# bjing2016/mdgen

Measured on AMD Instinct MI355X. Metric: sampled MD frames/sec, higher is better.
Workload: dtype bf16; 1 GPU; tetrapeptide_fwdsim_crop4_T1000_B16; batch_per_gpu=16, num_frames=1000, crop=4, euler_steps=49, hipgraph=True, parallelism=batch-sharded x1, no collective

## Files before the change

### mdgen_amd/csrc/k_gemm.hip

```cpp
#include "kernels.h"
#include "panel.h"

namespace mdg {

constexpr int kRowB = kC * 2;
constexpr int kPanelBytes = kPanel * kRowB;

constexpr int kRopeLds = kRopeRow + 4;
constexpr int kBiasUnits = 3 * kC / 4;
struct QkvStage {
    float bias[3][kC];
    float rope[kPanel][kRopeLds];
};
struct Attn4Stage {
    float bias[3][kC];
    uint32_t tab[2][kL4Tab];
    float rope[4][kRopeLds];
};
__device__ __forceinline__ const f32x4* stage_bias_src(const QkvParams& p, int u) {
    const float* b = u < kC / 4 ? p.bq : u < 2 * (kC / 4) ? p.bk : p.bv;
    return reinterpret_cast<const f32x4*>(b) + (u % (kC / 4));
}
template <int NT>
struct QkvStager {
// ... 296 lines not shown
        prologue_bf16<kC>(panel, pr, p.obuf);
        __syncthreads();
        wave_gemm<2, 3, 24, false, 4, true>(panel, kRowB, 0, 0, p.wo + (size_t)(3 * w) * 24 * 64 + lane, 24 * 64, acc);
        __syncthreads();
        epilogue_gate_residual_lds<3>(acc, pr, reinterpret_cast<float*>(panel) + w * (32 * 96), 96 * w, p.bo, p.mm, p.gate_chunk,
                                      true, p.h_rw);
        __syncthreads();
    }
    prologue_ln<false>(panel, pr, PRE ? p.h_rw : p.h, p.mm, p.shift_chunk, p.scale_chunk, 1e-6f);
    __syncthreads();
    QKV_STAMP(1);
    const int ntile = p.ax.ntile();
    const int len = p.ax.len;
    wave_gemm<2, 3, 24, true, 4, true>(panel, kRowB, 0, 0, p.wq + (size_t)(3 * w) * 24 * 64 + lane, 24 * 64, acc);
    QKV_STAMP(2);
    epilogue_heads_T<true, 2, !SMALL>(acc, pr, w, sbq, srope, SMALL, pos0, len, seq, ntile, tile0, p.qf, p.qkv_small, 0);
    __builtin_amdgcn_sched_barrier(0);
    QKV_STAMP(3);
    wave_gemm<2, 3, 24, true, 4, true>(panel, kRowB, 0, 0, p.wk + (size_t)(3 * w) * 24 * 64 + lane, 24 * 64, acc);
    QKV_STAMP(4);
    epilogue_heads_T<true, 2, !SMALL>(acc, pr, w, sbk, srope, SMALL, pos0, len, seq, ntile, tile0, p.kf, p.qkv_small, 1);
    __builtin_amdgcn_sched_barrier(0);
    QKV_STAMP(5);
    if (SMALL) {
        wave_gemm<2, 3, 24, true, 4, true>(panel, kRowB, 0, 0, p.wv + (size_t)(3 * w) * 24 * 64 + lane, 24 * 64, acc);
        epilogue_heads_T<false>(acc, pr, w, p.bv, nullptr, true, pos0, len, seq, ntile, tile0, nullptr, p.qkv_small, 2);
    } else {
        wave_gemm<2, 3, 24, false, 4, true>(panel, kRowB, 0, 0, p.wv + (size_t)(3 * w) * 24 * 64 + lane, 24 * 64, acc);
        QKV_STAMP(6);
        epilogue_v_flash(acc, w, sbv, seq, ntile, tile0, p.vf);
        if ((int)blockIdx.x - seq * p.panels_per_seq == p.panels_per_seq - 1) {
            __builtin_amdgcn_sched_barrier(0);
            write_bias_slots(p, seq, w);
        }
        QKV_STAMP(7);
    }
}

template <int J>
__device__ __forceinline__ float quad_bcast(float v) {
    return __builtin_bit_cast(float, __builtin_amdgcn_update_dpp(0, __builtin_bit_cast(int, v), J * 0x55, 0xf, 0xf, true));
}
template <int J>
__device__ __forceinline__ float fmac_dpp(float acc, float k, float q) {
    asm("v_fmac_f32_dpp %0, %1, %2 quad_perm:[%3,%3,%3,%3] row_mask:0xf bank_mask:0xf bound_ctrl:1" : "+v"(acc) : "v"(k), "v"(q), "n"(J));
    return acc;
}
template <int J>
__device__ __forceinline__ float mul_dpp(float k, float q) {
    float r;
    asm("v_mul_f32_dpp %0, %1, %2 quad_perm:[%3,%3,%3,%3] row_mask:0xf bank_mask:0xf bound_ctrl:1" : "=v"(r) : "v"(k), "v"(q), "n"(J));
    return r;
}
__device__ __forceinline__ void dpp_fence(float (&k)[12]) {
    asm volatile("s_nop 1"
                 : "+v"(k[0]), "+v"(k[1]), "+v"(k[2]), "+v"(k[3]), "+v"(k[4]), "+v"(k[5]), "+v"(k[6]), "+v"(k[7]), "+v"(k[8]), "+v"(k[9]),
                   "+v"(k[10]), "+v"(k[11]));
}
__device__ __forceinline__ float half_sum(float x) {
    const auto r = __builtin_amdgcn_permlane32_swap(__float_as_uint(x), __float_as_uint(x), false, false);
    return __uint_as_float(r[0]) + __uint_as_float(r[1]);
}
template <int TT = 2>
__device__ __forceinline__ void head_values(const f32x16* acc, int tt, int hd, const f32x4 (&bq)[3], float (&e)[12]) {
#pragma unroll
    for (int c = 0; c < 3; ++c) {
        const int ap = 3 * hd + c, ft = ap >> 2, a = ap & 3;
#pragma unroll
        for (int b = 0; b < 4; ++b) e[4 * c + b] = acc[ft * TT + tt][4 * a + b] + bq[c][b];
    }
}
template <bool X1S>
__device__ __forceinline__ void rotate_pair(float x1, float x2, float c, float sn, float& e0, float& e1) {
    const float a = x2 * sn;
    e0 = __builtin_fmaf(x1, c, -a);
    if (X1S) {
        const float b = x1 * sn;
        e1 = __builtin_fmaf(x2, c, b);
    } else {
        const float b = x2 * c;
        e1 = __builtin_fmaf(x1, sn, b);
    }
}
__device__ __forceinline__ void load_head_bias(const float* bias_perm, int w, int hh, f32x4 (&bq)[4][3]) {
    const f32x4* bp = reinterpret_cast<const f32x4*>(bias_perm + (w * 2 + hh) * 48);
#pragma unroll
    for (int hd = 0; hd < 4; ++hd)
#pragma unroll
        for (int c = 0; c < 3; ++c) bq[hd][c] = bp[hd * 3 + c];
}


template <bool SPLIT, bool HALF = false>
__global__ __launch_bounds__(512, 1) void k_ln_qkv8(const QkvParams p) {
    static_assert(!HALF || SPLIT, "32-row workgroups exist in the split form only");
    constexpr int TT = HALF ? 1 : 2, kRows = 32 * TT;
    __shared__ __attribute__((aligned(16))) unsigned char smem[sizeof(PanelRows) + kPanelBytes];
    __shared__ __attribute__((aligned(16))) QkvStage stage;
    QkvStager<512> stager;
    PanelRows* pr = reinterpret_cast<PanelRows*>(smem);
    unsigned char* panel = smem + sizeof(PanelRows);
    const int blk = SPLIT ? blockIdx.x >> 1 : blockIdx.x, half = SPLIT ? blockIdx.x & 1 : 0;
    const int seq = blk / p.panels_per_seq;
    const int pn = blk - seq * p.panels_per_seq;
    const int pos0 = pn * kRows, tile0 = pn * TT;
    stager.load(p, pos0, p.ax.len, threadIdx.x);
    setup_rows_axis(pr, p.ax, seq, pos0, p.mm, kRows);
    if (wave_id() == 0 && half == 0) {
        const int lane = lane_id(), len = p.ax.len, pos = pos0 + lane;
        const float mv = p.mk.at(p.ax.token(seq, pos < len ? pos : len - 1));
        const unsigned long long bal = __ballot(pos == len || (pos < len && mv != 0.f));
        uint32_t* vm = p.vmask + (long)seq * p.vmask_stride;
        if (lane < TT) vm[tile0 + lane] = (uint32_t)(bal >> (32 * lane));
        if (pn == p.panels_per_seq - 1) {
            const int idx = tile0 + TT + lane;
            if (idx < p.vmask_stride) vm[idx] = idx == (len >> 5) ? 1u << (len & 31) : 0u;
            if (idx + 64 < p.vmask_stride) vm[idx + 64] = 0u;
        }
    }
    __syncthreads();
    stager.store(&stage, threadIdx.x);
    const int w8 = __builtin_amdgcn_readfirstlane(wave_id()), g = w8 >> 2, w = w8 & 3, lane = lane_id();
    if (HALF) {
        if (g == 0) prologue_ln<false, 0, 1>(panel, pr, p.h, p.mm, p.shift_chunk, p.scale_chunk, 1e-6f, w, lane);
        else prologue_ln<false, 1, 2>(panel, pr, p.h, p.mm, p.shift_chunk, p.scale_chunk, 1e-6f, w, lane);
    } else {
        if (g == 0) prologue_ln<false, 0, 2>(panel, pr, p.h, p.mm, p.shift_chunk, p.scale_chunk, 1e-6f, w, lane);
        else prologue_ln<false, 2, 4>(panel, pr, p.h, p.mm, p.shift_chunk, p.scale_chunk, 1e-6f, w, lane);
    }
    __syncthreads();
    const int ntile = p.ax.ntile(), len = p.ax.len;
    const bool last = pn == p.panels_per_seq - 1;
    f32x16 acc[3 * TT];
    const bool do_q = SPLIT ? half == 0 && g == 0 : g == 0, do_k = SPLIT ? half == 0 && g == 1 : g == 0;
    const bool do_v = SPLIT ? half == 1 && g == 0 : g == 1;
    if (do_q) {
        wave_gemm<TT, 3, 24, true, 4, true>(panel, kRowB, 0, 0, p.wq + (size_t)(3 * w) * 24 * 64 + lane, 24 * 64, acc);
        epilogue_heads_T<true, TT, true>(acc, pr, w, stage.bias[0], &stage.rope[0][0], false, pos0, len, seq, ntile, tile0, p.qf, p.qkv_small, 0);
        __builtin_amdgcn_sched_barrier(0);
    }
    if (do_k) {
        wave_gemm<TT, 3, 24, true, 4, true>(panel, kRowB, 0, 0, p.wk + (size_t)(3 * w) * 24 * 64 + lane, 24 * 64, acc);
        epilogue_heads_T<true, TT, true>(acc, pr, w, stage.bias[1], &stage.rope[0][0], false, pos0, len, seq, ntile, tile0, p.kf, p.qkv_small, 1);
        if (last) {
            __builtin_amdgcn_sched_barrier(0);
            write_bias_slots(p, seq, w, true, false, TT);
        }
    }
    if (do_v) {
        wave_gemm<TT, 3, 24, false, 4, true>(panel, kRowB, 0, 0, p.wv + (size_t)(3 * w) * 24 * 64 + lane, 24 * 64, acc);
        epilogue_v_flash<TT>(acc, w, stage.bias[2], seq, ntile, tile0, p.vf);
        if (last) {
            __builtin_amdgcn_sched_barrier(0);
            write_bias_slots(p, seq, w, false, true, TT);
        }
    }
}

constexpr int kAttn4KPF = 2, kAttn4VPF = 3;
template <bool PROJ, bool HALF = false>
__global__ __launch_bounds__(256, 2) void k_ln_qkv_attn4(const QkvParams p) {
    static_assert(!HALF || PROJ, "the half-panel form is the whole sub-layer");
    constexpr int TT = HALF ? 1 : 2, kRows = HALF ? 32 : kPanel;
    __shared__ __attribute__((aligned(16))) unsigned char smem[sizeof(PanelRows) + kPanelBytes];
    __shared__ uint32_t qstash[HALF ? 1 : 4][24][64];
    __shared__ __attribute__((aligned(16))) Attn4Stage stage;
    Attn4Stager stager;
    PanelRows* pr = reinterpret_cast<PanelRows*>(smem);
    unsigned char* panel = smem + sizeof(PanelRows);
    ATTN4_STAMP_DECL;
    ATTN4_STAMP(0);
    stager.load(p, threadIdx.x);
    {
        const long row0 = (long)blockIdx.x * kRows, rend = row0 + kRows;
        setup_rows_linear(pr, row0, rend < p.nrows ? rend : p.nrows, p.mm);
    }
    __syncthreads();
    stager.store(&stage, threadIdx.x);
    const int w = __builtin_amdgcn_readfirstlane(wave_id());
    constexpr int t0 = 0;
    if (HALF) prologue_ln<false, 0, 2>(panel, pr, p.h, p.mm, p.shift_chunk, p.scale_chunk, 1e-6f, w, lane_id());
    else prologue_ln<false>(panel, pr, p.h, p.mm, p.shift_chunk, p.scale_chunk, 1e-6f);
    __syncthreads();
    ATTN4_STAMP(1);
    const int lane = lane_id(), hh = lane >> 5, tk = lane & 31;
    constexpr int L = 4;
    int tok[TT];
    float mval[TT];
#pragma unroll
    for (int tt = 0; tt < TT; ++tt) {
        tok[tt] = pr->tok[(t0 + tt) * 32 + tk];
        mval[tt] = p.mk.at(tok[tt] < 0 ? 0 : tok[tt]);
    }
    auto load_rope = [&](f32x4 (&rq)[TT][4]) {
#pragma unroll
        for (int tt = 0; tt < TT; ++tt) {
            const int tc = tok[tt] < 0 ? 0 : tok[tt];
            const f32x4* rc = reinterpret_cast<const f32x4*>(&stage.rope[tc & (L - 1)][16 * hh]);
#pragma unroll
            for (int i = 0; i < 4; ++i) rq[tt][i] = rc[i];
        }
    };
    f32x16 acc[3 * TT];
    f32x4 bb[4][3];
    f32x4 rq[TT][4];
    wave_gemm<TT, 3, 24, true, 4, true>(panel, kRowB, t0, 0, p.wq + (size_t)(3 * w) * 24 * 64 + lane, 24 * 64, acc);
    ATTN4_STAMP(2);
    load_head_bias(stage.bias[0], w, hh, bb);
    load_rope(rq);
    uint32_t qp[TT][4][6];
#pragma unroll
    for (int tt = 0; tt < TT; ++tt)
#pragma unroll
        for (int hd = 0; hd < 4; ++hd) {
            float e[12];
            head_values<TT>(acc, tt, hd, bb[hd], e);
#pragma unroll
            for (int q = 0; q < 6; ++q) {
                const float c = rq[tt][q >> 2][q & 3], sn = rq[tt][2 + (q >> 2)][q & 3];
                float r0, r1;
                rotate_pair<HALF>(e[2 * q], e[2 * q + 1], c, sn, r0, r1);
                qp[tt][hd][q] = pack_bf16(r0, r1);
            }
        }
    if constexpr (!HALF) {
#pragma unroll
        for (int hd = 0; hd < 4; ++hd)
#pragma unroll
            for (int q = 0; q < 6; ++q) qstash[w][hd * 6 + q][lane] = qp[TT - 1][hd][q];
    }
    ATTN4_STAMP(3);
    __builtin_amdgcn_sched_barrier(0);
    wave_gemm<TT, 3, 24, true, HALF ? 4 : kAttn4KPF, true>(panel, kRowB, t0, 0, p.wk + (size_t)(3 * w) * 24 * 64 + lane, 24 * 64, acc);
    ATTN4_STAMP(4);
    load_head_bias(stage.bias[1], w, hh, bb);
    load_rope(rq);
#pragma unroll
    for (int tt = 0; tt < TT; ++tt)
#pragma unroll
        for (int hd = 0; hd < 4; ++hd) {
            float k[12];
            head_values<TT>(acc, tt, hd, bb[hd], k);
#pragma unroll
            for (int c = 0; c < 3; ++c) {
                const int ap = 3 * hd + c, ft = ap >> 2, a = ap & 3;
#pragma unroll
                for (int b2 = 0; b2 < 2; ++b2) {
                    const int q = 2 * c + b2;
                    const float cs = rq[tt][q >> 2][q & 3], sn = rq[tt][2 + (q >> 2)][q & 3];
                    float r0, r1;
                    rotate_pair<HALF>(k[2 * q], k[2 * q + 1], cs, sn, r0, r1);
                    acc[ft * TT + tt][4 * a + 2 * b2] = r0;
                    acc[ft * TT + tt][4 * a + 2 * b2 + 1] = r1;
                }
            }
        }
    ATTN4_STAMP(5);
    __builtin_amdgcn_sched_barrier(0);
    float P[TT][4][5];
    {
#pragma unroll
        for (int hd = 0; hd < 4; ++hd) {
            const uint32_t* kt = &stage.tab[0][((2 * w + hh) * 4 + hd) * 6];
            float kb[12];
#pragma unroll
            for (int q = 0; q < 6; ++q) {
                kb[2 * q] = bf16_lo(kt[q]);
                kb[2 * q + 1] = bf16_hi(kt[q]);
            }
#pragma unroll
            for (int tt = 0; tt < TT; ++tt) {
                float k[12], qf[12];
#pragma unroll
                for (int c = 0; c < 3; ++c) {
                    const int ap = 3 * hd + c, ft = ap >> 2, a = ap & 3;
#pragma unroll
                    for (int b2 = 0; b2 < 4; ++b2) k[4 * c + b2] = acc[ft * TT + tt][4 * a + b2];
                }
#pragma unroll
                for (int q = 0; q < 6; ++q) {
                    const uint32_t u = (HALF || tt == 0) ? qp[tt][hd][q] : qstash[w][hd * 6 + q][lane];
                    qf[2 * q] = bf16_lo(u);
                    qf[2 * q + 1] = bf16_hi(u);
                }
                dpp_fence(k);
                float s[5];
                s[0] = mul_dpp<0>(k[0], qf[0]);
                s[1] = mul_dpp<1>(k[0], qf[0]);
                s[2] = mul_dpp<2>(k[0], qf[0]);
                s[3] = mul_dpp<3>(k[0], qf[0]);
                s[4] = 0.f;
#pragma unroll
                for (int i = 0; i < 12; ++i) {
                    if (i > 0) {
                        s[0] = fmac_dpp<0>(s[0], k[i], qf[i]);
                        s[1] = fmac_dpp<1>(s[1], k[i], qf[i]);
                        s[2] = fmac_dpp<2>(s[2], k[i], qf[i]);
                        s[3] = fmac_dpp<3>(s[3], k[i], qf[i]);
                    }
                    s[4] += qf[i] * kb[i];
                }
#pragma unroll
                for (int j = 0; j < 5; ++j) s[j] = half_sum(s[j]);
                const float m0 = quad_bcast<0>(mval[tt]), m1 = quad_bcast<1>(mval[tt]), m2 = quad_bcast<2>(mval[tt]),
                            m3 = quad_bcast<3>(mval[tt]);
                s[0] = m0 != 0.f ? s[0] : -1e30f;
                s[1] = m1 != 0.f ? s[1] : -1e30f;
                s[2] = m2 != 0.f ? s[2] : -1e30f;
                s[3] = m3 != 0.f ? s[3] : -1e30f;
                const float mx = fmaxf(fmaxf(fmaxf(s[0], s[1]), fmaxf(s[2], s[3])), s[4]);
                float den = 0.f;
#pragma unroll
                for (int j = 0; j < 5; ++j) {
                    s[j] = s[j] > -1e29f ? __builtin_amdgcn_exp2f(s[j] - mx) : 0.f;
                    den += s[j];
                }
                const float inv = 1.0f / den;
#pragma unroll
                for (int j = 0; j < 5; ++j) P[tt][hd][j] = s[j] * inv;
            }
            __builtin_amdgcn_sched_barrier(0);
        }
    }
    ATTN4_STAMP(6);
    uint32_t Pk[10];
    if constexpr (HALF) {
        const float* Pf = &P[0][0][0];
#pragma unroll
        for (int i = 0; i < 10; ++i) Pk[i] = pack_bf16(Pf[2 * i], Pf[2 * i + 1]);
    } else {
        const float* Pf = &P[0][0][0];
#pragma unroll
        for (int i = 0; i < 20; ++i) qstash[w][i][lane] = pack_bf16(Pf[2 * i], Pf[2 * i + 1]);
    }
    __builtin_amdgcn_sched_barrier(0);
    wave_gemm<TT, 3, 24, true, HALF ? 4 : kAttn4VPF, true>(panel, kRowB, t0, 0, p.wv + (size_t)(3 * w) * 24 * 64 + lane, 24 * 64, acc);
    ATTN4_STAMP(7);
    load_head_bias(stage.bias[2], w, hh, bb);
    {
        float* Pf = &P[0][0][0];
#pragma unroll
        for (int i = 0; i < 10 * TT; ++i) {
            const uint32_t u = HALF ? Pk[i % 10] : qstash[w][i][lane];
            Pf[2 * i] = bf16_lo(u);
            Pf[2 * i + 1] = bf16_hi(u);
        }
    }
    if (PROJ) __syncthreads();
#pragma unroll
    for (int hd = 0; hd < 4; ++hd) {
        const int head = 4 * w + hd;
        const uint32_t* vt = &stage.tab[1][((2 * w + hh) * 4 + hd) * 6];
        float bvv[12];
#pragma unroll
        for (int q = 0; q < 6; ++q) {
            bvv[2 * q] = bf16_lo(vt[q]);
            bvv[2 * q + 1] = bf16_hi(vt[q]);
        }
#pragma unroll
        for (int tt = 0; tt < TT; ++tt) {
            float v[12], o[12];
            head_values<TT>(acc, tt, hd, bb[hd], v);
            dpp_fence(v);
#pragma unroll
            for (int i = 0; i < 12; ++i) o[i] = mul_dpp<1>(v[i], P[tt][hd][1]);
#pragma unroll
            for (int i = 0; i < 12; ++i) o[i] = fmac_dpp<0>(o[i], v[i], P[tt][hd][0]);
#pragma unroll
            for (int i = 0; i < 12; ++i) o[i] = fmac_dpp<2>(o[i], v[i], P[tt][hd][2]);
#pragma unroll
            for (int i = 0; i < 12; ++i) o[i] = fmac_dpp<3>(o[i], v[i], P[tt][hd][3]);
#pragma unroll
            for (int i = 0; i < 12; ++i) o[i] = __builtin_fmaf(P[tt][hd][4], bvv[i], o[i]);
            if (PROJ) {
                const bool ok = tok[tt] >= 0;
#pragma unroll
                for (int i = 0; i < 3; ++i)
                    *reinterpret_cast<u32x2*>(panel + panel_off((t0 + tt) * 32 + tk, head * 48 + hh * 24 + 8 * i, kRowB)) =
                        u32x2{ok ? pack_bf16(o[4 * i], o[4 * i + 1]) : 0u, ok ? pack_bf16(o[4 * i + 2], o[4 * i + 3]) : 0u};
            } else if (tok[tt] >= 0) {
                u32x2* d = reinterpret_cast<u32x2*>(p.obuf + (long)tok[tt] * kC + head * kDH + hh * 12);
                d[0] = u32x2{pack_bf16(o[0], o[1]), pack_bf16(o[2], o[3])};
                d[1] = u32x2{pack_bf16(o[4], o[5]), pack_bf16(o[6], o[7])};
                d[2] = u32x2{pack_bf16(o[8], o[9]), pack_bf16(o[10], o[11])};
            }
        }
        __builtin_amdgcn_sched_barrier(0);
    }
    if (!PROJ) return;
    __syncthreads();
    ATTN4_STAMP(8);
    wave_gemm<TT, 3, 24, false, 4, true>(panel, kRowB, t0, 0, p.wo + (size_t)(3 * w) * 24 * 64 + lane, 24 * 64, acc);
    ATTN4_STAMP(9);
    __syncthreads();
    if constexpr (HALF) {
        float* stage = reinterpret_cast<float*>(panel) + w * (32 * 96);
        epi_stage(acc, stage);
        epi_rmw<8>(0, pr, stage, 96 * w, p.bo, p.mm, p.gate_chunk, true, p.h_rw);
    } else {
        epilogue_gate_residual_lds<3>(acc, pr, reinterpret_cast<float*>(panel) + w * (32 * 96), 96 * w, p.bo, p.mm, p.gate_chunk,
                                      true, p.h_rw);
    }
    ATTN4_STAMP(10);
    ATTN4_STAMP_FLUSH
}

template <int MAXL>
__device__ __forceinline__ void prologue_micro_attn(unsigned char* panel, const PanelRows* pr, const ProjParams& p) {
    const int L = p.ax.len;
    for (int item = threadIdx.x; item < kPanel * kH; item += 256) {
        const int row = item >> 4, head = item & 15;
        const int token = pr->tok[row];
        const int tkc = token < 0 ? 0 : token;
        const int seq = tkc / L;
        const __bf16* sbase = p.qkv_small + (long)seq * L * (3 * kC) + head * kDH;
        const u32x4* qp = reinterpret_cast<const u32x4*>(p.qkv_small + (long)tkc * (3 * kC) + head * kDH);
        u32x4 qv[3], kk[MAXL][3], vv[MAXL][3];
        float mk[MAXL];
#pragma unroll
        for (int i = 0; i < 3; ++i) qv[i] = qp[i];
#pragma unroll
        for (int j = 0; j < MAXL; ++j) {
            const int jc = j < L ? j : L - 1;
            mk[j] = p.mk.at((long)seq * L + jc);
            const u32x4* kp = reinterpret_cast<const u32x4*>(sbase + (long)jc * (3 * kC) + kC);
#pragma unroll
            for (int i = 0; i < 3; ++i) kk[j][i] = kp[i];
        }
        if (MAXL <= 4) {
#pragma unroll
            for (int j = 0; j < MAXL; ++j) {
                const int jc = j < L ? j : L - 1;
                const u32x4* vp = reinterpret_cast<const u32x4*>(sbase + (long)jc * (3 * kC) + 2 * kC);
#pragma unroll
                for (int i = 0; i < 3; ++i) vv[j][i] = vp[i];
            }
        }
        float q[24];
#pragma unroll
        for (int i = 0; i < 3; ++i)
#pragma unroll
            for (int j = 0; j < 4; ++j) {
                q[8 * i + 2 * j] = bf16_lo(qv[i][j]);
                q[8 * i + 2 * j + 1] = bf16_hi(qv[i][j]);
            }
        float s[MAXL + 1];
        float mx = -1e30f;
#pragma unroll
        for (int j = 0; j < MAXL; ++j) {
            float d = 0.f;
#pragma unroll
            for (int i = 0; i < 3; ++i)
#pragma unroll
                for (int jj = 0; jj < 4; ++jj)
                    d += q[8 * i + 2 * jj] * bf16_lo(kk[j][i][jj]) + q[8 * i + 2 * jj + 1] * bf16_hi(kk[j][i][jj]);
            s[j] = (j < L && mk[j] != 0.f) ? d : -1e30f;
// ... 631 lines not shown
```

### mdgen_amd/csrc/panel.h

```cpp
#pragma once
#include "common.h"

namespace mdg {

__device__ __forceinline__ void lds_barrier() { asm volatile("s_waitcnt lgkmcnt(0)\n\ts_barrier" ::: "memory"); }

__device__ __forceinline__ int panel_off(int row, int byte_in_row, int rowb) {
    return row * rowb + (byte_in_row ^ ((row & 15) << 4));
}

__device__ __forceinline__ bf16x8 panel_frag(const unsigned char* panel, const int rowb, int tile, int ks) {
    const int lane = lane_id();
    const int row = tile * 32 + (lane & 31);
    return *reinterpret_cast<const bf16x8*>(panel + panel_off(row, ks * 32 + (lane >> 5) * 16, rowb));
}

template <int TT, int FT, int KSTEPS, bool TRANS, int PF = 4, bool ZC = false>
__device__ __forceinline__ void wave_gemm(const unsigned char* panel, const int rowb, const int tile0, const int ks0,
                                          const bf16x8* __restrict__ wfrag, const int wtile_stride,
                                          f32x16* acc) {
    static_assert(PF < KSTEPS, "prefetch depth");
    bf16x8 wring[PF + 1][FT];
    bf16x8 aring[2][TT];
    const f32x16 zero = {0.f, 0.f, 0.f, 0.f, 0.f, 0.f, 0.f, 0.f, 0.f, 0.f, 0.f, 0.f, 0.f, 0.f, 0.f, 0.f};
#pragma unroll
    for (int p = 0; p < PF; ++p)
#pragma unroll
        for (int f = 0; f < FT; ++f) wring[p][f] = wfrag[(size_t)f * wtile_stride + p * 64];
#pragma unroll
    for (int t = 0; t < TT; ++t) aring[0][t] = panel_frag(panel, rowb, tile0 + t, ks0);
    __builtin_amdgcn_sched_barrier(0);
#pragma unroll
    for (int ks = 0; ks < KSTEPS; ++ks) {
        if (ks + PF < KSTEPS) {
#pragma unroll
            for (int f = 0; f < FT; ++f)
                wring[(ks + PF) % (PF + 1)][f] = wfrag[(size_t)f * wtile_stride + (ks + PF) * 64];
        }
        if (ks + 1 < KSTEPS) {
#pragma unroll
            for (int t = 0; t < TT; ++t) aring[(ks + 1) & 1][t] = panel_frag(panel, rowb, tile0 + t, ks0 + ks + 1);
        }
        __builtin_amdgcn_sched_barrier(0);
#pragma unroll
        for (int t = 0; t < TT; ++t)
#pragma unroll
            for (int f = 0; f < FT; ++f) {
                if (TRANS)
                    acc[f * TT + t] = __builtin_amdgcn_mfma_f32_32x32x16_bf16(wring[ks % (PF + 1)][f], aring[ks & 1][t],
                                                                             ZC && ks == 0 ? zero : acc[f * TT + t], 0, 0, 0);
                else
                    acc[t * FT + f] = __builtin_amdgcn_mfma_f32_32x32x16_bf16(aring[ks & 1][t], wring[ks % (PF + 1)][f],
                                                                             ZC && ks == 0 ? zero : acc[t * FT + f], 0, 0, 0);
            }
        if (ZC && ks == 0) {
#pragma unroll
            for (int t = 0; t < TT; ++t)
#pragma unroll
                for (int f = 0; f < FT; ++f)
                    asm volatile("" : "+v"(acc[TRANS ? f * TT + t : t * FT + f]) : "v"(wring[0][f]), "v"(aring[0][t]));
        }
        __builtin_amdgcn_sched_barrier(0);
    }
}

template <int N>
__device__ __forceinline__ void zero_acc(f32x16* acc) {
#pragma unroll
    for (int i = 0; i < N; ++i)
#pragma unroll
        for (int r = 0; r < 16; ++r) acc[i][r] = opaque_zero();
}

struct PanelRows {
    int tok[kPanel];
    int moff[kPanel];
    int uniform;
    int pad_[3];
};

__device__ __forceinline__ void set_uniform(PanelRows* pr, int tid, long t, long mo) {
    const int mo0 = __builtin_amdgcn_readfirstlane((int)mo);
    const int t0 = __builtin_amdgcn_readfirstlane((int)t);
    const bool same = t < 0 || (int)mo == mo0;
    const bool all = __builtin_amdgcn_ballot_w64(same) == ~0ull;
    if (tid == 0) pr->uniform = (t0 >= 0 && all) ? mo0 : -1;
}

__device__ __forceinline__ void setup_rows_axis(PanelRows* pr, const AxisMap ax, int seq, int pos0, const ModMap mm, int nrows = kPanel) {
    if (threadIdx.x < kPanel) {
        const int pos = pos0 + threadIdx.x;
        long t = -1, mo = 0;
        if (pos < ax.len && (int)threadIdx.x < nrows) {
            t = ax.token(seq, pos);
            mo = mm.row_off(t);
        }
        pr->tok[threadIdx.x] = (int)t;
// ... 87 lines not shown
#pragma unroll
            for (int i = 0; i < 3; ++i) {
                const float m0 = AFFINE ? sc[j][i][0] : 1.0f + sc[j][i][0];
                const float m1 = AFFINE ? sc[j][i][1] : 1.0f + sc[j][i][1];
                const float y0 = v[b][j][i][0] * rstd[j] * m0 + sh[j][i][0];
                const float y1 = v[b][j][i][1] * rstd[j] * m1 + sh[j][i][1];
                *reinterpret_cast<uint32_t*>(panel + panel_off(r0 + j, 4 * lane + 256 * i, ROWB)) =
                    t[b][j] >= 0 ? pack_bf16(y0, y1) : 0u;
            }
        }
    }
}

template <bool AFFINE, int B0 = 0, int B1 = 4>
__device__ __forceinline__ void prologue_ln(unsigned char* panel, const PanelRows* pr, const float* __restrict__ x,
                                            const ModMap mm, int shift_chunk, int scale_chunk, float eps,
                                            const int w = wave_id(), const int lane = lane_id()) {
    const int um = AFFINE ? 0 : pr->uniform;
    if (um >= 0) prologue_ln_impl<AFFINE, B0, B1, true>(panel, pr, x, mm, shift_chunk, scale_chunk, eps, w, lane, um);
    else prologue_ln_impl<AFFINE, B0, B1, false>(panel, pr, x, mm, shift_chunk, scale_chunk, eps, w, lane, 0);
}

template <int K>
__device__ __forceinline__ void prologue_bf16(unsigned char* panel, const PanelRows* pr, const __bf16* __restrict__ src) {
    constexpr int ROWB = K * 2;
    constexpr int CPR = ROWB / 16;
    constexpr int NIT = kPanel * CPR / 256;
    static_assert(kPanel * CPR % 256 == 0, "whole iterations");
    u32x4 v[NIT];
    int tk[NIT];
#pragma unroll
    for (int it = 0; it < NIT; ++it) {
        const int i = threadIdx.x + 256 * it;
        const int r = i / CPR, c = i % CPR;
        tk[it] = pr->tok[r];
        v[it] = *reinterpret_cast<const u32x4*>(reinterpret_cast<const unsigned char*>(src) +
                                                (long)(tk[it] < 0 ? 0 : tk[it]) * ROWB + c * 16);
    }
#pragma unroll
    for (int it = 0; it < NIT; ++it) {
        const int i = threadIdx.x + 256 * it;
        const int r = i / CPR, c = i % CPR;
        *reinterpret_cast<u32x4*>(panel + panel_off(r, c * 16, ROWB)) = tk[it] >= 0 ? v[it] : u32x4{0u, 0u, 0u, 0u};
    }
}

template <int TT, int FT>
__device__ __forceinline__ void epilogue_gate_residual(const f32x16* acc, const PanelRows* pr, int col0,
                                                       const float* __restrict__ bias, const ModMap mm,
                                                       int gate_chunk, bool gated, float* __restrict__ h) {
    const int lane = lane_id();
    const int hh = lane >> 5, n = lane & 31;
    float b[FT];
#pragma unroll
    for (int f = 0; f < FT; ++f) b[f] = bias[col0 + f * 32 + n];
#pragma unroll
    for (int t = 0; t < TT; ++t) {
#pragma unroll
        for (int r = 0; r < 16; ++r) {
            const int row = t * 32 + mfma_row(r, hh);
            const int tk = pr->tok[row];
            if (tk >= 0) {
                float* hp = h + (long)tk * kC + col0 + n;
                const float* gp = mm.mod + pr->moff[row] + gate_chunk * kC + col0 + n;
#pragma unroll
                for (int f = 0; f < FT; ++f) {
                    const float g = gated ? gp[f * 32] : 1.0f;
                    hp[f * 32] = hp[f * 32] + g * (acc[t * FT + f][r] + b[f]);
                }
            }
        }
    }
}

__device__ __forceinline__ void epi_stage(const f32x16* acc3, float* stage) {
    const int lane = lane_id();
    const int hh = lane >> 5, n = lane & 31;
#pragma unroll
    for (int f = 0; f < 3; ++f)
#pragma unroll
        for (int r = 0; r < 16; ++r) stage[mfma_row(r, hh) * 96 + f * 32 + n] = acc3[f][r];
}

template <int BR>
__device__ __forceinline__ void epi_rmw(const int t, const PanelRows* pr, const float* stage, int col0,
                                        const float* __restrict__ bias, const ModMap mm, int gate_chunk, bool gated,
                                        float* __restrict__ h, const PanelRows* prd = nullptr, float* hd = nullptr) {
    static_assert(16 % BR == 0, "batches of row pairs");
    const int lane = lane_id();
    const int q = lane % 24, r2 = lane / 24;
    const bool active = lane < 48;
    const int slot = active ? lane : 0;
    const f32x4 b4 = *reinterpret_cast<const f32x4*>(bias + col0 + 4 * q);
    const f32x4* stage4 = reinterpret_cast<const f32x4*>(stage);
    const int um = gated ? pr->uniform : -1;
    const bool per_row = gated && um < 0;
    f32x4 gu = f32x4{1.f, 1.f, 1.f, 1.f};
    if (gated && um >= 0) gu = *reinterpret_cast<const f32x4*>(mm.mod + um + gate_chunk * kC + col0 + 4 * q);
#pragma unroll
    for (int b = 0; b < 16 / BR; ++b) {
        f32x4 hv[BR], g[BR];
        int tk[BR], td[BR];
#pragma unroll
        for (int k = 0; k < BR; ++k) {
            const int row = active ? t * 32 + 2 * (BR * b + k) + r2 : 0;
            tk[k] = active ? pr->tok[row] : -1;
            td[k] = prd ? prd->tok[row] : tk[k];
            const long tc = tk[k] < 0 ? 0 : tk[k];
            hv[k] = *reinterpret_cast<const f32x4*>(h + tc * kC + col0 + 4 * q);
            g[k] = gu;
            if (per_row) g[k] = *reinterpret_cast<const f32x4*>(mm.mod + pr->moff[row] + gate_chunk * kC + col0 + 4 * q);
        }
#pragma unroll
        for (int k = 0; k < BR; ++k) {
            const f32x4 v = stage4[(BR * b + k) * 48 + slot];
            f32x4 o = hv[k];
            o[0] += g[k][0] * (v[0] + b4[0]);
            o[1] += g[k][1] * (v[1] + b4[1]);
            o[2] += g[k][2] * (v[2] + b4[2]);
            o[3] += g[k][3] * (v[3] + b4[3]);
            if (tk[k] >= 0) *reinterpret_cast<f32x4*>((hd ? hd : h) + (long)td[k] * kC + col0 + 4 * q) = o;
        }
    }
}

template <int BR>
struct EpiPre {
    f32x4 hv[BR];
    int tk[BR];
};
template <int BR>
__device__ __forceinline__ void epi_rmw_request(const int t, const int b, const PanelRows* pr, int col0, const float* __restrict__ h,
                                                EpiPre<BR>& e) {
    const int lane = lane_id();
    const int q = lane % 24, r2 = lane / 24;
    const bool active = lane < 48;
#pragma unroll
    for (int k = 0; k < BR; ++k) {
        const int row = active ? t * 32 + 2 * (BR * b + k) + r2 : 0;
        e.tk[k] = active ? pr->tok[row] : -1;
        const long tc = e.tk[k] < 0 ? 0 : e.tk[k];
        e.hv[k] = *reinterpret_cast<const f32x4*>(h + tc * kC + col0 + 4 * q);
    }
}
template <int BR>
__device__ __forceinline__ void epi_rmw_finish(const int b, const float* stage, int col0, const f32x4 b4, const f32x4 gu,
                                               float* __restrict__ h, const EpiPre<BR>& e) {
    const int lane = lane_id();
    const int q = lane % 24;
    const int slot = lane < 48 ? lane : 0;
    const f32x4* stage4 = reinterpret_cast<const f32x4*>(stage);
#pragma unroll
    for (int k = 0; k < BR; ++k) {
        const f32x4 v = stage4[(BR * b + k) * 48 + slot];
        f32x4 o = e.hv[k];
        o[0] += gu[0] * (v[0] + b4[0]);
        o[1] += gu[1] * (v[1] + b4[1]);
        o[2] += gu[2] * (v[2] + b4[2]);
        o[3] += gu[3] * (v[3] + b4[3]);
        if (e.tk[k] >= 0) *reinterpret_cast<f32x4*>(h + (long)e.tk[k] * kC + col0 + 4 * q) = o;
    }
}
template <int FT>
__device__ __forceinline__ void epilogue_gate_residual_lds_pre(const f32x16* acc, const PanelRows* pr, float* stage, int col0,
                                                               const float* __restrict__ bias, const ModMap mm, int gate_chunk,
                                                               bool gated, float* __restrict__ h, EpiPre<8>& e0) {
    static_assert(FT == 3, "slab is [32][96]");
    const int um = gated ? pr->uniform : -1;
    if (um < 0) {
#pragma unroll
        for (int t = 0; t < 2; ++t) {
            epi_stage(acc + t * FT, stage);
            epi_rmw<8>(t, pr, stage, col0, bias, mm, gate_chunk, gated, h);
        }
        return;
    }
    const int q = lane_id() % 24;
    const f32x4 b4 = *reinterpret_cast<const f32x4*>(bias + col0 + 4 * q);
    const f32x4 gu = *reinterpret_cast<const f32x4*>(mm.mod + um + gate_chunk * kC + col0 + 4 * q);
    EpiPre<8> e1;
    epi_stage(acc, stage);
    epi_rmw_request<8>(0, 1, pr, col0, h, e1);
    __builtin_amdgcn_sched_barrier(0);
    epi_rmw_finish<8>(0, stage, col0, b4, gu, h, e0);
    __builtin_amdgcn_sched_barrier(0);
    epi_rmw_request<8>(1, 0, pr, col0, h, e0);
    __builtin_amdgcn_sched_barrier(0);
    epi_rmw_finish<8>(1, stage, col0, b4, gu, h, e1);
    __builtin_amdgcn_sched_barrier(0);
    epi_stage(acc + FT, stage);
    epi_rmw_request<8>(1, 1, pr, col0, h, e1);
    __builtin_amdgcn_sched_barrier(0);
    epi_rmw_finish<8>(0, stage, col0, b4, gu, h, e0);
    __builtin_amdgcn_sched_barrier(0);
    epi_rmw_finish<8>(1, stage, col0, b4, gu, h, e1);
}

template <int FT>
__device__ __forceinline__ void epilogue_gate_residual_lds(const f32x16* acc, const PanelRows* pr, float* stage, int col0,
                                                           const float* __restrict__ bias, const ModMap mm,
                                                           int gate_chunk, bool gated, float* __restrict__ h) {
    static_assert(FT == 3, "slab is [32][96]");
#pragma unroll
    for (int t = 0; t < 2; ++t) {
        epi_stage(acc + t * FT, stage);
        epi_rmw<8>(t, pr, stage, col0, bias, mm, gate_chunk, gated, h);
    }
}

}
```

Measured before the change: 125,400 frames/s.

## Scope attention-kernel temporaries per head and spread epilogue across all lanes

The fused LN+QKV attention kernel now loads bias and rope values per head and per token tile instead of holding them in full register arrays. It packs softmax probabilities to bf16 as each head finishes, rather than keeping a whole float P array alive across the V GEMM. The intent is to reduce register pressure and spills. The residual epilogue is remapped so all 64 lanes do work instead of 48, and panel_frag addressing changes for k-steps beyond 8. These changes alter LDS indexing and stash layout, which risks subtle correctness or bank-conflict effects.

```diff
diff --git a/mdgen_amd/csrc/k_gemm.hip b/mdgen_amd/csrc/k_gemm.hip
--- a/mdgen_amd/csrc/k_gemm.hip
+++ b/mdgen_amd/csrc/k_gemm.hip
@@ -402,12 +402,10 @@
         e1 = __builtin_fmaf(x1, sn, b);
     }
 }
-__device__ __forceinline__ void load_head_bias(const float* bias_perm, int w, int hh, f32x4 (&bq)[4][3]) {
-    const f32x4* bp = reinterpret_cast<const f32x4*>(bias_perm + (w * 2 + hh) * 48);
-#pragma unroll
-    for (int hd = 0; hd < 4; ++hd)
-#pragma unroll
-        for (int c = 0; c < 3; ++c) bq[hd][c] = bp[hd * 3 + c];
+__device__ __forceinline__ void load_head_bias(const float* bias_perm, int w, int hh, int hd, f32x4 (&bq)[3]) {
+    const f32x4* bp = reinterpret_cast<const f32x4*>(bias_perm + (w * 2 + hh) * 48) + hd * 3;
+#pragma unroll
+    for (int c = 0; c < 3; ++c) bq[c] = bp[c];
 }
 
 
@@ -512,62 +510,59 @@
         tok[tt] = pr->tok[(t0 + tt) * 32 + tk];
         mval[tt] = p.mk.at(tok[tt] < 0 ? 0 : tok[tt]);
     }
-    auto load_rope = [&](f32x4 (&rq)[TT][4]) {
-#pragma unroll
-        for (int tt = 0; tt < TT; ++tt) {
-            const int tc = tok[tt] < 0 ? 0 : tok[tt];
-            const f32x4* rc = reinterpret_cast<const f32x4*>(&stage.rope[tc & (L - 1)][16 * hh]);
-#pragma unroll
-            for (int i = 0; i < 4; ++i) rq[tt][i] = rc[i];
-        }
+    auto load_rope = [&](int tt, f32x4 (&rq)[4]) {
+        const int tc = tok[tt] < 0 ? 0 : tok[tt];
+        const f32x4* rc = reinterpret_cast<const f32x4*>(&stage.rope[tc & (L - 1)][16 * hh]);
+#pragma unroll
+        for (int i = 0; i < 4; ++i) rq[i] = rc[i];
     };
     f32x16 acc[3 * TT];
-    f32x4 bb[4][3];
-    f32x4 rq[TT][4];
     wave_gemm<TT, 3, 24, true, 4, true>(panel, kRowB, t0, 0, p.wq + (size_t)(3 * w) * 24 * 64 + lane, 24 * 64, acc);
     ATTN4_STAMP(2);
-    load_head_bias(stage.bias[0], w, hh, bb);
-    load_rope(rq);
-    uint32_t qp[TT][4][6];
-#pragma unroll
-    for (int tt = 0; tt < TT; ++tt)
+    uint32_t qp[4][6];
+#pragma unroll
+    for (int tt = TT - 1; tt >= 0; --tt) {
+        f32x4 rq[4];
+        load_rope(tt, rq);
 #pragma unroll
         for (int hd = 0; hd < 4; ++hd) {
+            f32x4 bq[3];
+            load_head_bias(stage.bias[0], w, hh, hd, bq);
             float e[12];
-            head_values<TT>(acc, tt, hd, bb[hd], e);
+            head_values<TT>(acc, tt, hd, bq, e);
 #pragma unroll
             for (int q = 0; q < 6; ++q) {
-                const float c = rq[tt][q >> 2][q & 3], sn = rq[tt][2 + (q >> 2)][q & 3];
+                const float c = rq[q >> 2][q & 3], sn = rq[2 + (q >> 2)][q & 3];
                 float r0, r1;
                 rotate_pair<HALF>(e[2 * q], e[2 * q + 1], c, sn, r0, r1);
-                qp[tt][hd][q] = pack_bf16(r0, r1);
-            }
-        }
-    if constexpr (!HALF) {
-#pragma unroll
-        for (int hd = 0; hd < 4; ++hd)
-#pragma unroll
-            for (int q = 0; q < 6; ++q) qstash[w][hd * 6 + q][lane] = qp[TT - 1][hd][q];
+                uint32_t u = pack_bf16(r0, r1);
+                asm("" : "+v"(u));
+                if (tt == 0) qp[hd][q] = u;
+                else qstash[w][hd * 6 + q][lane] = u;
+            }
+        }
     }
     ATTN4_STAMP(3);
     __builtin_amdgcn_sched_barrier(0);
     wave_gemm<TT, 3, 24, true, HALF ? 4 : kAttn4KPF, true>(panel, kRowB, t0, 0, p.wk + (size_t)(3 * w) * 24 * 64 + lane, 24 * 64, acc);
     ATTN4_STAMP(4);
-    load_head_bias(stage.bias[1], w, hh, bb);
-    load_rope(rq);
-#pragma unroll
-    for (int tt = 0; tt < TT; ++tt)
+#pragma unroll
+    for (int tt = 0; tt < TT; ++tt) {
+        f32x4 rq[4];
+        load_rope(tt, rq);
 #pragma unroll
         for (int hd = 0; hd < 4; ++hd) {
+            f32x4 bq[3];
+            load_head_bias(stage.bias[1], w, hh, hd, bq);
             float k[12];
-            head_values<TT>(acc, tt, hd, bb[hd], k);
+            head_values<TT>(acc, tt, hd, bq, k);
 #pragma unroll
             for (int c = 0; c < 3; ++c) {
                 const int ap = 3 * hd + c, ft = ap >> 2, a = ap & 3;
 #pragma unroll
                 for (int b2 = 0; b2 < 2; ++b2) {
                     const int q = 2 * c + b2;
-                    const float cs = rq[tt][q >> 2][q & 3], sn = rq[tt][2 + (q >> 2)][q & 3];
+                    const float cs = rq[q >> 2][q & 3], sn = rq[2 + (q >> 2)][q & 3];
                     float r0, r1;
                     rotate_pair<HALF>(k[2 * q], k[2 * q + 1], cs, sn, r0, r1);
                     acc[ft * TT + tt][4 * a + 2 * b2] = r0;
@@ -575,9 +570,11 @@
                 }
             }
         }
+    }
     ATTN4_STAMP(5);
     __builtin_amdgcn_sched_barrier(0);
-    float P[TT][4][5];
+    uint32_t Pk[10];
+    float p4even = 0.f;
     {
 #pragma unroll
         for (int hd = 0; hd < 4; ++hd) {
@@ -588,6 +585,7 @@
                 kb[2 * q] = bf16_lo(kt[q]);
                 kb[2 * q + 1] = bf16_hi(kt[q]);
             }
+            float Pw[TT][5];
 #pragma unroll
             for (int tt = 0; tt < TT; ++tt) {
                 float k[12], qf[12];
@@ -599,7 +597,7 @@
                 }
 #pragma unroll
                 for (int q = 0; q < 6; ++q) {
-                    const uint32_t u = (HALF || tt == 0) ? qp[tt][hd][q] : qstash[w][hd * 6 + q][lane];
+                    const uint32_t u = tt == 0 ? qp[hd][q] : qstash[w][hd * 6 + q][lane];
                     qf[2 * q] = bf16_lo(u);
                     qf[2 * q + 1] = bf16_hi(u);
                 }
@@ -637,35 +635,33 @@
                 }
                 const float inv = 1.0f / den;
 #pragma unroll
-                for (int j = 0; j < 5; ++j) P[tt][hd][j] = s[j] * inv;
+                for (int j = 0; j < 5; ++j) Pw[tt][j] = s[j] * inv;
+            }
+            if constexpr (HALF) {
+                Pk[2 * hd] = pack_bf16(Pw[0][0], Pw[0][1]);
+                Pk[2 * hd + 1] = pack_bf16(Pw[0][2], Pw[0][3]);
+                asm("" : "+v"(Pk[2 * hd]), "+v"(Pk[2 * hd + 1]));
+                if (hd & 1) {
+                    Pk[8 + hd / 2] = pack_bf16(p4even, Pw[0][4]);
+                    asm("" : "+v"(Pk[8 + hd / 2]));
+                } else {
+                    p4even = Pw[0][4];
+                }
+            } else {
+#pragma unroll
+                for (int tt = 0; tt < TT; ++tt) {
+                    qstash[w][6 * hd + 3 * tt][lane] = pack_bf16(Pw[tt][0], Pw[tt][1]);
+                    qstash[w][6 * hd + 3 * tt + 1][lane] = pack_bf16(Pw[tt][2], Pw[tt][3]);
+                    qstash[w][6 * hd + 3 * tt + 2][lane] = pack_bf16(Pw[tt][4], 0.f);
+                }
             }
             __builtin_amdgcn_sched_barrier(0);
         }
     }
     ATTN4_STAMP(6);
-    uint32_t Pk[10];
-    if constexpr (HALF) {
-        const float* Pf = &P[0][0][0];
-#pragma unroll
-        for (int i = 0; i < 10; ++i) Pk[i] = pack_bf16(Pf[2 * i], Pf[2 * i + 1]);
-    } else {
-        const float* Pf = &P[0][0][0];
-#pragma unroll
-        for (int i = 0; i < 20; ++i) qstash[w][i][lane] = pack_bf16(Pf[2 * i], Pf[2 * i + 1]);
-    }
     __builtin_amdgcn_sched_barrier(0);
     wave_gemm<TT, 3, 24, true, HALF ? 4 : kAttn4VPF, true>(panel, kRowB, t0, 0, p.wv + (size_t)(3 * w) * 24 * 64 + lane, 24 * 64, acc);
     ATTN4_STAMP(7);
-    load_head_bias(stage.bias[2], w, hh, bb);
-    {
-        float* Pf = &P[0][0][0];
-#pragma unroll
-        for (int i = 0; i < 10 * TT; ++i) {
-            const uint32_t u = HALF ? Pk[i % 10] : qstash[w][i][lane];
-            Pf[2 * i] = bf16_lo(u);
-            Pf[2 * i + 1] = bf16_hi(u);
-        }
-    }
     if (PROJ) __syncthreads();
 #pragma unroll
     for (int hd = 0; hd < 4; ++hd) {
@@ -677,21 +673,33 @@
             bvv[2 * q] = bf16_lo(vt[q]);
             bvv[2 * q + 1] = bf16_hi(vt[q]);
         }
+        f32x4 bq[3];
+        load_head_bias(stage.bias[2], w, hh, hd, bq);
 #pragma unroll
         for (int tt = 0; tt < TT; ++tt) {
-            float v[12], o[12];
-            head_values<TT>(acc, tt, hd, bb[hd], v);
+            float v[12], o[12], P[5];
+            {
+                const uint32_t u0 = HALF ? Pk[2 * hd] : qstash[w][6 * hd + 3 * tt][lane];
+                const uint32_t u1 = HALF ? Pk[2 * hd + 1] : qstash[w][6 * hd + 3 * tt + 1][lane];
+                const uint32_t u2 = HALF ? Pk[8 + hd / 2] : qstash[w][6 * hd + 3 * tt + 2][lane];
+                P[0] = bf16_lo(u0);
+                P[1] = bf16_hi(u0);
+                P[2] = bf16_lo(u1);
+                P[3] = bf16_hi(u1);
+                P[4] = (HALF && (hd & 1)) ? bf16_hi(u2) : bf16_lo(u2);
+            }
+            head_values<TT>(acc, tt, hd, bq, v);
             dpp_fence(v);
 #pragma unroll
-            for (int i = 0; i < 12; ++i) o[i] = mul_dpp<1>(v[i], P[tt][hd][1]);
-#pragma unroll
-            for (int i = 0; i < 12; ++i) o[i] = fmac_dpp<0>(o[i], v[i], P[tt][hd][0]);
-#pragma unroll
-            for (int i = 0; i < 12; ++i) o[i] = fmac_dpp<2>(o[i], v[i], P[tt][hd][2]);
-#pragma unroll
-            for (int i = 0; i < 12; ++i) o[i] = fmac_dpp<3>(o[i], v[i], P[tt][hd][3]);
-#pragma unroll
-            for (int i = 0; i < 12; ++i) o[i] = __builtin_fmaf(P[tt][hd][4], bvv[i], o[i]);
+            for (int i = 0; i < 12; ++i) o[i] = mul_dpp<1>(v[i], P[1]);
+#pragma unroll
+            for (int i = 0; i < 12; ++i) o[i] = fmac_dpp<0>(o[i], v[i], P[0]);
+#pragma unroll
+            for (int i = 0; i < 12; ++i) o[i] = fmac_dpp<2>(o[i], v[i], P[2]);
+#pragma unroll
+            for (int i = 0; i < 12; ++i) o[i] = fmac_dpp<3>(o[i], v[i], P[3]);
+#pragma unroll
+            for (int i = 0; i < 12; ++i) o[i] = __builtin_fmaf(P[4], bvv[i], o[i]);
             if (PROJ) {
                 const bool ok = tok[tt] >= 0;
 #pragma unroll
diff --git a/mdgen_amd/csrc/panel.h b/mdgen_amd/csrc/panel.h
--- a/mdgen_amd/csrc/panel.h
+++ b/mdgen_amd/csrc/panel.h
@@ -12,7 +12,7 @@
 __device__ __forceinline__ bf16x8 panel_frag(const unsigned char* panel, const int rowb, int tile, int ks) {
     const int lane = lane_id();
     const int row = tile * 32 + (lane & 31);
-    return *reinterpret_cast<const bf16x8*>(panel + panel_off(row, ks * 32 + (lane >> 5) * 16, rowb));
+    return *reinterpret_cast<const bf16x8*>(panel + panel_off(row, (ks & 7) * 32 + (lane >> 5) * 16, rowb) + (ks >> 3) * 256);
 }
 
 template <int TT, int FT, int KSTEPS, bool TRANS, int PF = 4, bool ZC = false>
@@ -266,83 +266,107 @@
         for (int r = 0; r < 16; ++r) stage[mfma_row(r, hh) * 96 + f * 32 + n] = acc3[f][r];
 }
 
+struct EpiLane {
+    int q[3], r[3];
+    __device__ __forceinline__ EpiLane() {
+        const int lane = lane_id();
+#pragma unroll
+        for (int j = 0; j < 3; ++j) {
+            const int x = lane + 16 * j;
+            r[j] = 2 * j + x / 24;
+            q[j] = x % 24;
+        }
+    }
+    __device__ __forceinline__ int row(int i) const { return 8 * (i / 3) + r[i % 3]; }
+    __device__ __forceinline__ int col(int i) const { return 4 * q[i % 3]; }
+};
+__device__ __forceinline__ void epi_load3(const float* v, const EpiLane& el, f32x4 (&o)[3]) {
+#pragma unroll
+    for (int j = 0; j < 3; ++j) o[j] = *reinterpret_cast<const f32x4*>(v + 4 * el.q[j]);
+}
+
 template <int BR>
 __device__ __forceinline__ void epi_rmw(const int t, const PanelRows* pr, const float* stage, int col0,
                                         const float* __restrict__ bias, const ModMap mm, int gate_chunk, bool gated,
                                         float* __restrict__ h, const PanelRows* prd = nullptr, float* hd = nullptr) {
-    static_assert(16 % BR == 0, "batches of row pairs");
+    static_assert(16 % BR == 0 && BR % 4 == 0, "batches of row pairs, whole items");
+    constexpr int NI = 3 * BR / 4;
     const int lane = lane_id();
-    const int q = lane % 24, r2 = lane / 24;
-    const bool active = lane < 48;
-    const int slot = active ? lane : 0;
-    const f32x4 b4 = *reinterpret_cast<const f32x4*>(bias + col0 + 4 * q);
+    const EpiLane el;
+    f32x4 b4[3];
+    epi_load3(bias + col0, el, b4);
     const f32x4* stage4 = reinterpret_cast<const f32x4*>(stage);
     const int um = gated ? pr->uniform : -1;
     const bool per_row = gated && um < 0;
-    f32x4 gu = f32x4{1.f, 1.f, 1.f, 1.f};
-    if (gated && um >= 0) gu = *reinterpret_cast<const f32x4*>(mm.mod + um + gate_chunk * kC + col0 + 4 * q);
+    f32x4 gu[3] = {f32x4{1.f, 1.f, 1.f, 1.f}, f32x4{1.f, 1.f, 1.f, 1.f}, f32x4{1.f, 1.f, 1.f, 1.f}};
+    if (gated && um >= 0) epi_load3(mm.mod + um + gate_chunk * kC + col0, el, gu);
 #pragma unroll
     for (int b = 0; b < 16 / BR; ++b) {
-        f32x4 hv[BR], g[BR];
-        int tk[BR], td[BR];
-#pragma unroll
-        for (int k = 0; k < BR; ++k) {
-            const int row = active ? t * 32 + 2 * (BR * b + k) + r2 : 0;
-            tk[k] = active ? pr->tok[row] : -1;
+        f32x4 hv[NI], g[NI];
+        int tk[NI], td[NI];
+#pragma unroll
+        for (int k = 0; k < NI; ++k) {
+            const int i = NI * b + k, row = t * 32 + el.row(i);
+            tk[k] = pr->tok[row];
             td[k] = prd ? prd->tok[row] : tk[k];
             const long tc = tk[k] < 0 ? 0 : tk[k];
-            hv[k] = *reinterpret_cast<const f32x4*>(h + tc * kC + col0 + 4 * q);
-            g[k] = gu;
-            if (per_row) g[k] = *reinterpret_cast<const f32x4*>(mm.mod + pr->moff[row] + gate_chunk * kC + col0 + 4 * q);
-        }
-#pragma unroll
-        for (int k = 0; k < BR; ++k) {
-            const f32x4 v = stage4[(BR * b + k) * 48 + slot];
+            hv[k] = *reinterpret_cast<const f32x4*>(h + tc * kC + col0 + el.col(i));
+            g[k] = gu[i % 3];
+            if (per_row) g[k] = *reinterpret_cast<const f32x4*>(mm.mod + pr->moff[row] + gate_chunk * kC + col0 + el.col(i));
+        }
+#pragma unroll
+        for (int k = 0; k < NI; ++k) {
+            const int i = NI * b + k;
+            const f32x4 v = stage4[64 * i + lane];
+            const f32x4 bi = b4[i % 3];
             f32x4 o = hv[k];
-            o[0] += g[k][0] * (v[0] + b4[0]);
-            o[1] += g[k][1] * (v[1] + b4[1]);
-            o[2] += g[k][2] * (v[2] + b4[2]);
-            o[3] += g[k][3] * (v[3] + b4[3]);
-            if (tk[k] >= 0) *reinterpret_cast<f32x4*>((hd ? hd : h) + (long)td[k] * kC + col0 + 4 * q) = o;
+            o[0] += g[k][0] * (v[0] + bi[0]);
+            o[1] += g[k][1] * (v[1] + bi[1]);
+            o[2] += g[k][2] * (v[2] + bi[2]);
+            o[3] += g[k][3] * (v[3] + bi[3]);
+            if (tk[k] >= 0) *reinterpret_cast<f32x4*>((hd ? hd : h) + (long)td[k] * kC + col0 + el.col(i)) = o;
         }
     }
 }
 
 template <int BR>
 struct EpiPre {
-    f32x4 hv[BR];
-    int tk[BR];
+    static_assert(16 % BR == 0 && BR % 4 == 0, "batches of row pairs, whole items");
+    static constexpr int NI = 3 * BR / 4;
+    f32x4 hv[NI];
+    int tk[NI];
 };
 template <int BR>
 __device__ __forceinline__ void epi_rmw_request(const int t, const int b, const PanelRows* pr, int col0, const float* __restrict__ h,
                                                 EpiPre<BR>& e) {
+    constexpr int NI = EpiPre<BR>::NI;
+    const EpiLane el;
+#pragma unroll
+    for (int k = 0; k < NI; ++k) {
+        const int i = NI * b + k;
+        e.tk[k] = pr->tok[t * 32 + el.row(i)];
+        const long tc = e.tk[k] < 0 ? 0 : e.tk[k];
+        e.hv[k] = *reinterpret_cast<const f32x4*>(h + tc * kC + col0 + el.col(i));
+    }
+}
+template <int BR>
+__device__ __forceinline__ void epi_rmw_finish(const int b, const float* stage, int col0, const f32x4 (&b4)[3], const f32x4 (&gu)[3],
+                                               float* __restrict__ h, const EpiPre<BR>& e) {
+    constexpr int NI = EpiPre<BR>::NI;
     const int lane = lane_id();
-    const int q = lane % 24, r2 = lane / 24;
-    const bool active = lane < 48;
-#pragma unroll
-    for (int k = 0; k < BR; ++k) {
-        const int row = active ? t * 32 + 2 * (BR * b + k) + r2 : 0;
-        e.tk[k] = active ? pr->tok[row] : -1;
-        const long tc = e.tk[k] < 0 ? 0 : e.tk[k];
-        e.hv[k] = *reinterpret_cast<const f32x4*>(h + tc * kC + col0 + 4 * q);
-    }
-}
-template <int BR>
-__device__ __forceinline__ void epi_rmw_finish(const int b, const float* stage, int col0, const f32x4 b4, const f32x4 gu,
-                                               float* __restrict__ h, const EpiPre<BR>& e) {
-    const int lane = lane_id();
-    const int q = lane % 24;
-    const int slot = lane < 48 ? lane : 0;
+    const EpiLane el;
     const f32x4* stage4 = reinterpret_cast<const f32x4*>(stage);
 #pragma unroll
-    for (int k = 0; k < BR; ++k) {
-        const f32x4 v = stage4[(BR * b + k) * 48 + slot];
+    for (int k = 0; k < NI; ++k) {
+        const int i = NI * b + k;
+        const f32x4 v = stage4[64 * i + lane];
+        const f32x4 bi = b4[i % 3], gi = gu[i % 3];
         f32x4 o = e.hv[k];
-        o[0] += gu[0] * (v[0] + b4[0]);
-        o[1] += gu[1] * (v[1] + b4[1]);
-        o[2] += gu[2] * (v[2] + b4[2]);
-        o[3] += gu[3] * (v[3] + b4[3]);
-        if (e.tk[k] >= 0) *reinterpret_cast<f32x4*>(h + (long)e.tk[k] * kC + col0 + 4 * q) = o;
+        o[0] += gi[0] * (v[0] + bi[0]);
+        o[1] += gi[1] * (v[1] + bi[1]);
+        o[2] += gi[2] * (v[2] + bi[2]);
+        o[3] += gi[3] * (v[3] + bi[3]);
+        if (e.tk[k] >= 0) *reinterpret_cast<f32x4*>(h + (long)e.tk[k] * kC + col0 + el.col(i)) = o;
     }
 }
 template <int FT>
@@ -359,9 +383,10 @@
         }
         return;
     }
-    const int q = lane_id() % 24;
-    const f32x4 b4 = *reinterpret_cast<const f32x4*>(bias + col0 + 4 * q);
-    const f32x4 gu = *reinterpret_cast<const f32x4*>(mm.mod + um + gate_chunk * kC + col0 + 4 * q);
+    const EpiLane el;
+    f32x4 b4[3], gu[3];
+    epi_load3(bias + col0, el, b4);
+    epi_load3(mm.mod + um + gate_chunk * kC + col0, el, gu);
     EpiPre<8> e1;
     epi_stage(acc, stage);
     epi_rmw_request<8>(0, 1, pr, col0, h, e1);
```

New measurement: 126,400 frames/s, median of 6. No clear change (+0.8%).
